# xuekt98/BBDM

Hardware: NVIDIA H100
Metric: denoising-steps/sec (UNet fwd) at 256^2 pixel-BBDM (higher is better)
Workload: dtype bf16x3 (split-bf16 tensor-core products, fp32 accumulate: fp32-class)

## Files before the change

bbdm_b200/csrc/winograd.cu:

```cuda
#include "common.cuh"
#include <cuda_fp16.h>
#include <stdlib.h>

namespace bbdm {

constexpr float WINO_WSCALE_FIXED = 256.0f;

__host__ __device__ inline float wino_wscale(uint32_t mbits) {
  if (mbits == 0) return WINO_WSCALE_FIXED;
  const int e = (int)(mbits >> 23) - 127;
  int k = 14 - (e + ((mbits & 0x7fffffu) != 0 ? 1 : 0));
  k = k < -100 ? -100 : (k > 100 ? 100 : k);
  float s = 1.0f;
  for (; k > 0; --k) s *= 2.0f;
  for (; k < 0; ++k) s *= 0.5f;
  return s;
}

template <int S>
__device__ __forceinline__ void wino_bt6(float* d) {
  const float d0 = d[0], d1 = d[S], d2 = d[2 * S], d3 = d[3 * S], d4 = d[4 * S], d5 = d[5 * S];
  d[0] = fmaf(4.0f, d0, fmaf(-5.0f, d2, d4));
  d[S] = fmaf(-4.0f, d1 + d2, d3 + d4);
  d[2 * S] = fmaf(4.0f, d1 - d2, d4 - d3);
  d[3 * S] = fmaf(2.0f, d3 - d1, d4 - d2);
  d[4 * S] = fmaf(2.0f, d1 - d3, d4 - d2);
  d[5 * S] = fmaf(4.0f, d1, fmaf(-5.0f, d3, d5));
}
template <int S, int T>
__host__ __device__ __forceinline__ void wino_at6(const float* m, float* y) {
  const float s12 = m[S] + m[2 * S], d12 = m[S] - m[2 * S];
  const float s34 = m[3 * S] + m[4 * S], d34 = m[3 * S] - m[4 * S];
  y[0] = (m[0] + s12) + s34;
  y[T] = fmaf(2.0f, d34, d12);
  y[2 * T] = fmaf(4.0f, s34, s12);
  y[3 * T] = fmaf(8.0f, d34, d12) + m[5 * S];
}

template <int S>
__device__ __forceinline__ void wino_bt8(float* d) {
  const float d0 = d[0], d1 = d[S], d2 = d[2 * S], d3 = d[3 * S], d4 = d[4 * S], d5 = d[5 * S], d6 = d[6 * S],
              d7 = d[7 * S];
  const float e1 = fmaf(-4.25f, d4, d2 + d6), o1 = fmaf(-4.25f, d3, d1 + d5);
  const float e3 = fmaf(0.25f, d2, fmaf(-1.25f, d4, d6)), o3 = fmaf(0.5f, d1, fmaf(-2.5f, d3, 2.0f * d5));
  const float e5 = fmaf(4.0f, d2, fmaf(-5.0f, d4, d6)), o5 = fmaf(2.0f, d1, fmaf(-2.5f, d3, 0.5f * d5));
  d[0] = fmaf(5.25f, d4 - d2, d0 - d6);
  d[S] = e1 + o1;
  d[2 * S] = e1 - o1;
  d[3 * S] = e3 + o3;
  d[4 * S] = e3 - o3;
  d[5 * S] = e5 + o5;
  d[6 * S] = e5 - o5;
  d[7 * S] = fmaf(5.25f, d3 - d5, d7 - d1);
}
template <int S, int T>
__host__ __device__ __forceinline__ void wino_at8(const float* m, float* y) {
  const float a = m[S] + m[2 * S], b = m[S] - m[2 * S];
  const float c = m[3 * S] + m[4 * S], d = m[3 * S] - m[4 * S];
  const float e = m[5 * S] + m[6 * S], f = m[5 * S] - m[6 * S];
  y[0] = ((m[0] + a) + c) + e;
  y[T] = fmaf(2.0f, d, fmaf(0.5f, f, b));
  y[2 * T] = fmaf(4.0f, c, fmaf(0.25f, e, a));
  y[3 * T] = fmaf(8.0f, d, fmaf(0.125f, f, b));
  y[4 * T] = fmaf(16.0f, c, fmaf(0.0625f, e, a));
  y[5 * T] = fmaf(32.0f, d, fmaf(0.03125f, f, b)) + m[7 * S];
}

__device__ __forceinline__ void split2_f16(float a, float b, uint32_t& hi, uint32_t& lo) {
  const __half2 h = __floats2half2_rn(a, b);
  const float2 hf = __half22float2(h);
  const __half2 l = __floats2half2_rn(a - hf.x, b - hf.y);
  hi = *reinterpret_cast<const uint32_t*>(&h);
  lo = *reinterpret_cast<const uint32_t*>(&l);
}

struct WinoInParams {
  const float* src1; int c1;
  const float* src2; int c2;
  int B, H, W, C, groups, cpg, th, tw;
  int64_t Mtot;
  const float* mean; const float* rstd; const float* gamma; const float* beta;
  const float* fscale; const float* fshift; int64_t fstride;
  int silu;
  __half* v_hi; __half* v_lo;
  __nv_bfloat16* raw_hi; __nv_bfloat16* raw_lo;
  __nv_bfloat16* act_hi; __nv_bfloat16* act_lo;
  unsigned long long* fault;
};

constexpr unsigned long long WINO6_RANGE_FAULT = 0xC0000000ull;

template <int VEC>
__global__ void __launch_bounds__(256)
wino_input_kernel(const WinoInParams p) {
  const int b = blockIdx.x / p.th, ty = blockIdx.x % p.th;
  const int c = (blockIdx.y * 256 + threadIdx.x) * VEC;
  if (c >= p.C) return;
  float sc[VEC], sh[VEC];
#pragma unroll
  for (int v = 0; v < VEC; ++v) {
    const int g = (c + v) / p.cpg;
    const float s0 = p.rstd[b * p.groups + g] * p.gamma[c + v];
    const float h0 = p.beta[c + v] - p.mean[b * p.groups + g] * s0;
    float f1 = 1.0f, f0 = 0.0f;
    if (p.fscale) { f1 = 1.0f + p.fscale[(int64_t)b * p.fstride + c + v]; f0 = p.fshift[(int64_t)b * p.fstride + c + v]; }
    sc[v] = s0 * f1;
    sh[v] = fmaf(h0, f1, f0);
  }
  const float* base;
  int cs, cc;
  if (c < p.c1) { base = p.src1; cs = p.c1; cc = c; } else { base = p.src2; cs = p.c2; cc = c - p.c1; }
  const int y0 = 4 * ty - 1;
  float act[VEC][36];
  auto fill = [&](int x0, int j0) {
#pragma unroll
    for (int i = 0; i < 6; ++i) {
      const int iy = y0 + i;
#pragma unroll
      for (int j = 0; j < 6; ++j) {
        if (j < j0) continue;
        const int ix = x0 + j;
        const bool in = iy >= 0 && iy < p.H && ix >= 0 && ix < p.W;
        float x[VEC];
#pragma unroll
        for (int v = 0; v < VEC; ++v) x[v] = 0.f;
        if (in) {
          const float* ptr = base + (((int64_t)b * p.H + iy) * p.W + ix) * cs + cc;
          if (VEC == 2) { const float2 t = *reinterpret_cast<const float2*>(ptr); x[0] = t.x; x[VEC - 1] = t.y; }
          else x[0] = *ptr;
        }
        if (p.raw_hi && i >= 1 && i <= 4 && j >= 2) {
          const int64_t off = (((int64_t)b * p.H + iy) * p.W + ix) * p.C + c;
          if (in) {
            if (VEC == 2) {
              uint32_t h, l;
              split2x(x[0], x[VEC - 1], h, l);
              *reinterpret_cast<uint32_t*>(p.raw_hi + off) = h;
              *reinterpret_cast<uint32_t*>(p.raw_lo + off) = l;
            } else {
              split_bf16(x[0], p.raw_hi[off], p.raw_lo[off]);
            }
          }
        } else if (p.raw_hi && i >= 1 && i <= 4 && j == 1 && j0 == 0 && in) {
          const int64_t off = (((int64_t)b * p.H + iy) * p.W + ix) * p.C + c;
          if (VEC == 2) {
            uint32_t h, l;
            split2x(x[0], x[VEC - 1], h, l);
            *reinterpret_cast<uint32_t*>(p.raw_hi + off) = h;
            *reinterpret_cast<uint32_t*>(p.raw_lo + off) = l;
          } else {
            split_bf16(x[0], p.raw_hi[off], p.raw_lo[off]);
          }
        }
#pragma unroll
        for (int v = 0; v < VEC; ++v) {
          float a = fmaf(x[v], sc[v], sh[v]);
          if (p.silu) a = __fdividef(a, 1.0f + __expf(-a));
          act[v][i * 6 + j] = in ? a : 0.f;
        }
      }
    }
  };
  for (int tx = 0; tx < p.tw; ++tx) {
    if (tx == 0) fill(-1, 0);
    else {
#pragma unroll
      for (int v = 0; v < VEC; ++v)
#pragma unroll
        for (int i = 0; i < 6; ++i) { act[v][i * 6] = act[v][i * 6 + 4]; act[v][i * 6 + 1] = act[v][i * 6 + 5]; }
      fill(4 * tx - 1, 2);
    }
    float t[VEC][36];
#pragma unroll
    for (int v = 0; v < VEC; ++v) {
#pragma unroll
      for (int q = 0; q < 36; ++q) t[v][q] = act[v][q];
#pragma unroll
      for (int j = 0; j < 6; ++j) wino_bt6<6>(t[v] + j);
#pragma unroll
      for (int i = 0; i < 6; ++i) wino_bt6<1>(t[v] + 6 * i);
    }
    const int64_t m = ((int64_t)b * p.th + ty) * p.tw + tx;
#pragma unroll
    for (int q = 0; q < 36; ++q) {
      const int64_t off = ((int64_t)q * p.Mtot + m) * p.C + c;
      if (VEC == 2) {
        uint32_t h, l;
        split2_f16(t[0][q], t[VEC - 1][q], h, l);
        *reinterpret_cast<uint32_t*>(p.v_hi + off) = h;
        *reinterpret_cast<uint32_t*>(p.v_lo + off) = l;
      } else {
        const __half h = __float2half_rn(t[0][q]);
        p.v_hi[off] = h;
        p.v_lo[off] = __float2half_rn(t[0][q] - __half2float(h));
      }
    }
  }
}

template <int T>
struct WinoIn {
  static constexpr int N = T + 2;
  static constexpr int CC = 64;
  static constexpr int TX = T == 4 ? 8 : 4;
  static constexpr int COLS = T * TX + 2;
  static constexpr int PATCH = N * COLS * CC;
  static constexpr size_t SMEM = 2 * (size_t)PATCH * sizeof(float);
};
static_assert(WinoIn<4>::SMEM == 2 * 6 * 34 * 64 * 4 && WinoIn<6>::SMEM * 2 <= 227 * 1024, "staged patch budget");

__device__ __forceinline__ void cp_async16(uint32_t saddr, const void* g) {
  asm volatile("cp.async.cg.shared.global [%0], [%1], 16;" ::"r"(saddr), "l"(g) : "memory");
}

template <int T>
__global__ void __launch_bounds__(256, 2)
wino_input_smem_kernel(const WinoInParams p) {
  using K = WinoIn<T>;
  constexpr int N = K::N, CC = K::CC, TX = K::TX, COLS = K::COLS;
  extern __shared__ __align__(16) float patch[];
  const int b = blockIdx.x / p.th, ty = blockIdx.x % p.th;
  const int cbase = blockIdx.y * CC;
  const float* base;
  int cs, cc0;
  if (cbase < p.c1) { base = p.src1; cs = p.c1; cc0 = cbase; } else { base = p.src2; cs = p.c2; cc0 = cbase - p.c1; }
  const int y0 = T * ty - 1;
  const int tid = threadIdx.x;
  const int ch4 = tid & 15;
  const int pix0 = tid >> 4;
  constexpr int NPIX = N * COLS;

  if constexpr (T == 6) {
    if (blockIdx.x == 0) {
      const int64_t tiles = (int64_t)p.B * p.th * p.tw;
      const int npad = (int)(p.Mtot - tiles);
      for (int k = tid; k < N * N * npad * CC; k += 256) {
        const int c = k % CC, r = (k / CC) % npad, q = k / (CC * npad);
        const int64_t off = ((int64_t)q * p.Mtot + tiles + r) * p.C + cbase + c;
        p.v_hi[off] = __float2half_rn(0.f);
        p.v_lo[off] = __float2half_rn(0.f);
      }
    }
  }

  float sc[4], sh[4];
#pragma unroll
  for (int v = 0; v < 4; ++v) {
    sc[v] = 1.0f; sh[v] = 0.0f;
    if (p.mean) {
      const int c = cbase + ch4 * 4 + v;
      const int g = c / p.cpg;
      const float s0 = p.rstd[b * p.groups + g] * p.gamma[c];
      const float h0 = p.beta[c] - p.mean[b * p.groups + g] * s0;
      float f1 = 1.0f, f0 = 0.0f;
      if (p.fscale) { f1 = 1.0f + p.fscale[(int64_t)b * p.fstride + c]; f0 = p.fshift[(int64_t)b * p.fstride + c]; }
      sc[v] = s0 * f1;
      sh[v] = fmaf(h0, f1, f0);
    }
  }
  const int nseg = (p.tw + TX - 1) / TX;
  const uint32_t patch_s = (uint32_t)__cvta_generic_to_shared(patch);

  auto stage = [&](int seg, int buf) {
    const int x0 = T * TX * seg - 1;
    int i = 0, j = pix0;
    for (int px = pix0; px < NPIX; px += 16, j += 16) {
      if (j >= COLS) { j -= COLS; ++i; }
      const int iy = y0 + i, ix = x0 + j;
      if (iy >= 0 && iy < p.H && ix >= 0 && ix < p.W)
        cp_async16(patch_s + (uint32_t)(((buf * NPIX + px) * CC + ch4 * 4) * 4),
                   base + (((int64_t)b * p.H + iy) * p.W + ix) * cs + cc0 + ch4 * 4);
    }
    asm volatile("cp.async.commit_group;" ::: "memory");
  };

  stage(0, 0);
  for (int seg = 0; seg < nseg; ++seg) {
    const int buf = seg & 1;
    if (seg + 1 < nseg) {
      stage(seg + 1, buf ^ 1);
      asm volatile("cp.async.wait_group 1;" ::: "memory");
    } else {
      asm volatile("cp.async.wait_group 0;" ::: "memory");
    }
    __syncthreads();
    float* pb = patch + buf * K::PATCH;
    const int x0 = T * TX * seg - 1;
    int i = 0, j = pix0;
    for (int px = pix0; px < NPIX; px += 16, j += 16) {
      if (j >= COLS) { j -= COLS; ++i; }
      const int iy = y0 + i, ix = x0 + j;
      float4* q = reinterpret_cast<float4*>(pb + px * CC + ch4 * 4);
      float4 a = make_float4(0.f, 0.f, 0.f, 0.f);
      if (iy >= 0 && iy < p.H && ix >= 0 && ix < p.W) {
        const float4 x = *q;
        if (p.raw_hi && i >= 1 && i <= T && j >= 1 && j <= T * TX) {
          uint2 h, l;
          split4(x, h, l);
          const int64_t off = (((int64_t)b * p.H + iy) * p.W + ix) * p.C + cbase + ch4 * 4;
          *reinterpret_cast<uint2*>(p.raw_hi + off) = h;
          *reinterpret_cast<uint2*>(p.raw_lo + off) = l;
        }
        a.x = fmaf(x.x, sc[0], sh[0]); a.y = fmaf(x.y, sc[1], sh[1]);
        a.z = fmaf(x.z, sc[2], sh[2]); a.w = fmaf(x.w, sc[3], sh[3]);
        if (p.silu) {
          a.x = __fdividef(a.x, 1.0f + __expf(-a.x)); a.y = __fdividef(a.y, 1.0f + __expf(-a.y));
          a.z = __fdividef(a.z, 1.0f + __expf(-a.z)); a.w = __fdividef(a.w, 1.0f + __expf(-a.w));
        }
        if (p.act_hi && i >= 1 && i <= T && j >= 1 && j <= T * TX) {
          uint2 h, l;
          split4(a, h, l);
          const int64_t off = (((int64_t)b * p.H + iy) * p.W + ix) * p.C + cbase + ch4 * 4;
          *reinterpret_cast<uint2*>(p.act_hi + off) = h;
          *reinterpret_cast<uint2*>(p.act_lo + off) = l;
        }
      }
      *q = a;
    }
    __syncthreads();
    const int64_t plane = p.Mtot * p.C;
    if constexpr (T == 4) {
      const int txl = tid >> 5, c0 = (tid & 31) * 2;
      const int tx = TX * seg + txl;
      if (tx < p.tw) {
        float t0[36], t1[36];
#pragma unroll
        for (int i = 0; i < 6; ++i)
#pragma unroll
          for (int j = 0; j < 6; ++j) {
            const float2 v = *reinterpret_cast<const float2*>(pb + ((i * COLS + 4 * txl + j) * CC + c0));
            t0[i * 6 + j] = v.x;
            t1[i * 6 + j] = v.y;
          }
#pragma unroll
        for (int j = 0; j < 6; ++j) { wino_bt6<6>(t0 + j); wino_bt6<6>(t1 + j); }
#pragma unroll
        for (int i = 0; i < 6; ++i) { wino_bt6<1>(t0 + 6 * i); wino_bt6<1>(t1 + 6 * i); }
        const int64_t m = ((int64_t)b * p.th + ty) * p.tw + tx;
        __half* ph = p.v_hi + m * p.C + cbase + c0;
        __half* pl = p.v_lo + m * p.C + cbase + c0;
#pragma unroll
        for (int q = 0; q < 36; ++q) {
          uint32_t h, l;
          split2_f16(t0[q], t1[q], h, l);
          *reinterpret_cast<uint32_t*>(ph) = h;
          *reinterpret_cast<uint32_t*>(pl) = l;
          ph += plane;
          pl += plane;
        }
      }
    } else {
      const int txl = tid >> 6, c = tid & 63;
      const int tx = TX * seg + txl;
      if (tx < p.tw) {
        float t[64];
#pragma unroll
        for (int i = 0; i < 8; ++i)
#pragma unroll
          for (int j = 0; j < 8; ++j) t[i * 8 + j] = pb[(i * COLS + 6 * txl + j) * CC + c];
#pragma unroll
        for (int j = 0; j < 8; ++j) wino_bt8<8>(t + j);
#pragma unroll
        for (int i = 0; i < 8; ++i) wino_bt8<1>(t + 8 * i);
        const int64_t m = ((int64_t)b * p.th + ty) * p.tw + tx;
        __half* ph = p.v_hi + m * p.C + cbase + c;
        __half* pl = p.v_lo + m * p.C + cbase + c;
        bool finite = true;
#pragma unroll
        for (int q = 0; q < 64; ++q) {
          const __half h = __float2half_rn(t[q]);
          finite &= fabsf(t[q]) < 65520.0f;
          *ph = h;
          *pl = __float2half_rn(t[q] - __half2float(h));
          ph += plane;
          pl += plane;
        }
        if (!finite) atomicExch(p.fault, WINO6_RANGE_FAULT | (unsigned)(p.C & 0xFFFFFFF));
      }
    }
    __syncthreads();
  }
}

struct WinoOutParams {
  const float* m; int64_t Mtot;
  const float* inv_wscale;
  int B, H, W, Cout, th, tw;
  const float* bias;
  const float* residual; int res_mode;
  float* out;
  float* stats;
};

template <int RES>
__host__ __device__ __forceinline__ void wino_output_tile(const WinoOutParams& p, int b, int ty, int tx, int c, float2 bv,
                                                          float inv, float& sum0, float& sum1, float& sq0, float& sq1) {
  const int64_t m = ((int64_t)b * p.th + ty) * p.tw + tx;
  float mx[36], my[36];
#pragma unroll
  for (int q = 0; q < 36; ++q) {
    const float2 v = *reinterpret_cast<const float2*>(p.m + ((int64_t)q * p.Mtot + m) * p.Cout + c);
    mx[q] = v.x; my[q] = v.y;
  }
  constexpr int NRES = RES == BBDM_RES_NONE ? 1 : (RES == BBDM_RES_UP2 ? 4 : 16);
  float2 rs[NRES];
  if constexpr (RES == BBDM_RES_SAME) {
#pragma unroll
    for (int i = 0; i < 4; ++i)
#pragma unroll
      for (int j = 0; j < 4; ++j)
        rs[i * 4 + j] = *reinterpret_cast<const float2*>(
            p.residual + (((int64_t)b * p.H + 4 * ty + i) * p.W + 4 * tx + j) * p.Cout + c);
  } else if constexpr (RES == BBDM_RES_UP2) {
#pragma unroll
    for (int i = 0; i < 2; ++i)
#pragma unroll
      for (int j = 0; j < 2; ++j)
        rs[i * 2 + j] = *reinterpret_cast<const float2*>(
            p.residual + (((int64_t)b * (p.H >> 1) + 2 * ty + i) * (p.W >> 1) + 2 * tx + j) * p.Cout + c);
  } else if constexpr (RES == BBDM_RES_DOWN2) {
    const int64_t W2 = (int64_t)p.W * 2;
#pragma unroll
    for (int i = 0; i < 4; ++i)
#pragma unroll
      for (int j = 0; j < 4; ++j) {
        const float* rp = p.residual + (((int64_t)b * p.H * 2 + (4 * ty + i) * 2) * W2 + (4 * tx + j) * 2) * p.Cout + c;
        const float2 t0 = *reinterpret_cast<const float2*>(rp), t1 = *reinterpret_cast<const float2*>(rp + p.Cout);
        const float2 t2 = *reinterpret_cast<const float2*>(rp + W2 * p.Cout);
        const float2 t3 = *reinterpret_cast<const float2*>(rp + (W2 + 1) * p.Cout);
        rs[i * 4 + j] = make_float2(0.25f * (((t0.x + t1.x) + t2.x) + t3.x), 0.25f * (((t0.y + t1.y) + t2.y) + t3.y));
      }
  }
  float tx4[24], ty4[24], yx[16], yy[16];
#pragma unroll
  for (int j = 0; j < 6; ++j) { wino_at6<6, 6>(mx + j, tx4 + j); wino_at6<6, 6>(my + j, ty4 + j); }
#pragma unroll
  for (int i = 0; i < 4; ++i) { wino_at6<1, 1>(tx4 + 6 * i, yx + 4 * i); wino_at6<1, 1>(ty4 + 6 * i, yy + 4 * i); }
#pragma unroll
  for (int i = 0; i < 4; ++i) {
    const int hh = 4 * ty + i;
#pragma unroll
    for (int j = 0; j < 4; ++j) {
      const int ww = 4 * tx + j;
      float r0 = fmaf(yx[i * 4 + j], inv, bv.x), r1 = fmaf(yy[i * 4 + j], inv, bv.y);
      if constexpr (RES == BBDM_RES_SAME || RES == BBDM_RES_DOWN2) {
        r0 += rs[i * 4 + j].x; r1 += rs[i * 4 + j].y;
      } else if constexpr (RES == BBDM_RES_UP2) {
        r0 += rs[(i >> 1) * 2 + (j >> 1)].x; r1 += rs[(i >> 1) * 2 + (j >> 1)].y;
      }
      *reinterpret_cast<float2*>(p.out + (((int64_t)b * p.H + hh) * p.W + ww) * p.Cout + c) = make_float2(r0, r1);
      sum0 += r0; sum1 += r1;
      sq0 = fmaf(r0, r0, sq0); sq1 = fmaf(r1, r1, sq1);
    }
  }
}

template <int RES>
__global__ void __launch_bounds__(256, 2)
wino_output_kernel(const WinoOutParams p) {
  __shared__ float red[8][64][2];
  const int cg = blockIdx.x, ty = blockIdx.y, b = blockIdx.z;
  const int lane = threadIdx.x & 31, tl = threadIdx.x >> 5;
  const int c = cg * 64 + lane * 2;
  float2 bv = make_float2(0.f, 0.f);
  if (p.bias) bv = *reinterpret_cast<const float2*>(p.bias + c);
  const float inv = p.inv_wscale ? __ldg(p.inv_wscale) : 1.0f / WINO_WSCALE_FIXED;
  float sum0 = 0.f, sum1 = 0.f, sq0 = 0.f, sq1 = 0.f;
  for (int tx = tl; tx < p.tw; tx += 8) wino_output_tile<RES>(p, b, ty, tx, c, bv, inv, sum0, sum1, sq0, sq1);
  if (p.stats) {
    red[tl][lane * 2][0] = sum0; red[tl][lane * 2][1] = sq0;
    red[tl][lane * 2 + 1][0] = sum1; red[tl][lane * 2 + 1][1] = sq1;
    __syncthreads();
    if (threadIdx.x < 64) {
      float a = 0.f, q = 0.f;
#pragma unroll
      for (int k = 0; k < 8; ++k) { a += red[k][threadIdx.x][0]; q += red[k][threadIdx.x][1]; }
      const int64_t prow = (int64_t)b * p.th + ty;
      *reinterpret_cast<float2*>(p.stats + (prow * p.Cout + cg * 64 + threadIdx.x) * 2) = make_float2(a, q);
    }
  }
}

template <int RES>
__host__ __device__ __forceinline__ void wino6_output_tile(const WinoOutParams& p, int b, int ty, int tx, int c, float bv,
                                                           float inv, float& sum, float& sq) {
  const int64_t m = ((int64_t)b * p.th + ty) * p.tw + tx;
  float mm[64];
#pragma unroll
  for (int q = 0; q < 64; ++q) mm[q] = p.m[((int64_t)q * p.Mtot + m) * p.Cout + c];
  float t6[48], y[36];
#pragma unroll
  for (int j = 0; j < 8; ++j) wino_at8<8, 8>(mm + j, t6 + j);
#pragma unroll
  for (int i = 0; i < 6; ++i) wino_at8<1, 1>(t6 + 8 * i, y + 6 * i);
  const int h0 = 6 * ty, w0 = 6 * tx;
  float rup[RES == BBDM_RES_UP2 ? 9 : 1];
  if constexpr (RES == BBDM_RES_UP2) {
    const int H2 = p.H >> 1, W2 = p.W >> 1;
#pragma unroll
    for (int i = 0; i < 3; ++i)
#pragma unroll
      for (int j = 0; j < 3; ++j)
        rup[i * 3 + j] = 3 * ty + i < H2 && 3 * tx + j < W2
                             ? p.residual[(((int64_t)b * H2 + 3 * ty + i) * W2 + 3 * tx + j) * p.Cout + c] : 0.f;
  }
  const int64_t pix0 = ((int64_t)b * p.H + h0) * p.W + w0;
#pragma unroll
  for (int i0 = 0; i0 < 6; i0 += 3) {
    float rs[18];
#pragma unroll
    for (int i = 0; i < 3; ++i)
#pragma unroll
      for (int j = 0; j < 6; ++j) {
        rs[i * 6 + j] = 0.f;
        if (h0 + i0 + i >= p.H || w0 + j >= p.W) continue;
        if constexpr (RES == BBDM_RES_SAME) {
          rs[i * 6 + j] = p.residual[(pix0 + (int64_t)(i0 + i) * p.W + j) * p.Cout + c];
        } else if constexpr (RES == BBDM_RES_DOWN2) {
          const int64_t W2 = (int64_t)p.W * 2;
          const float* rp = p.residual + (((int64_t)b * p.H * 2 + (h0 + i0 + i) * 2) * W2 + (w0 + j) * 2) * p.Cout + c;
          rs[i * 6 + j] = 0.25f * (((rp[0] + rp[p.Cout]) + rp[W2 * p.Cout]) + rp[(W2 + 1) * p.Cout]);
        }
      }
#pragma unroll
    for (int i = 0; i < 3; ++i)
#pragma unroll
      for (int j = 0; j < 6; ++j) {
        if (h0 + i0 + i >= p.H || w0 + j >= p.W) continue;
        float r = fmaf(y[(i0 + i) * 6 + j], inv, bv);
        if constexpr (RES == BBDM_RES_SAME || RES == BBDM_RES_DOWN2) r += rs[i * 6 + j];
        else if constexpr (RES == BBDM_RES_UP2) r += rup[((i0 + i) >> 1) * 3 + (j >> 1)];
        p.out[(pix0 + (int64_t)(i0 + i) * p.W + j) * p.Cout + c] = r;
        sum += r;
        sq = fmaf(r, r, sq);
      }
  }
}

template <int RES>
__global__ void __launch_bounds__(256, RES == BBDM_RES_SAME || RES == BBDM_RES_DOWN2 ? 1 : 2)
wino6_output_kernel(const WinoOutParams p) {
  __shared__ float red[4][64][2];
  const int cg = blockIdx.x, ty = blockIdx.y, b = blockIdx.z;
  const int cl = threadIdx.x & 63, tl = threadIdx.x >> 6;
  const int c = cg * 64 + cl;
  const float bv = p.bias ? p.bias[c] : 0.f;
  const float inv = p.inv_wscale ? __ldg(p.inv_wscale) : 1.0f / WINO_WSCALE_FIXED;
  float sum = 0.f, sq = 0.f;
  for (int tx = tl; tx < p.tw; tx += 4) wino6_output_tile<RES>(p, b, ty, tx, c, bv, inv, sum, sq);
  if (p.stats) {
    red[tl][cl][0] = sum; red[tl][cl][1] = sq;
    __syncthreads();
    if (threadIdx.x < 64) {
      float a = 0.f, q = 0.f;
#pragma unroll
      for (int k = 0; k < 4; ++k) { a += red[k][threadIdx.x][0]; q += red[k][threadIdx.x][1]; }
      const int64_t prow = (int64_t)b * p.th + ty;
      *reinterpret_cast<float2*>(p.stats + (prow * p.Cout + cg * 64 + threadIdx.x) * 2) = make_float2(a, q);
    }
  }
}

__global__ void __launch_bounds__(256)
wino_wmax_kernel(const float* __restrict__ w, int64_t n, uint32_t* __restrict__ wmax) {
  uint32_t m = 0;
  for (int64_t i = (int64_t)blockIdx.x * blockDim.x + threadIdx.x; i < n; i += (int64_t)gridDim.x * blockDim.x)
    m = max(m, __float_as_uint(fabsf(w[i])));
#pragma unroll
  for (int o = 16; o > 0; o >>= 1) m = max(m, __shfl_xor_sync(0xffffffffu, m, o));
  if ((threadIdx.x & 31) == 0 && m) atomicMax(wmax, m);
}

__global__ void wino_wscale_store_kernel(float* inv) {
  *inv = 1.0f / wino_wscale(__float_as_uint(*inv));
}

template <int T>
__device__ __forceinline__ void wino_g(double g0, double g1, double g2, double* u) {
  if constexpr (T == 4) {
    u[0] = g0 / 4.0;
    u[1] = -(g0 + g1 + g2) / 6.0;
    u[2] = -(g0 - g1 + g2) / 6.0;
    u[3] = g0 / 24.0 + g1 / 12.0 + g2 / 6.0;
    u[4] = g0 / 24.0 - g1 / 12.0 + g2 / 6.0;
    u[5] = g2;
  } else {
    u[0] = g0;
    u[1] = -2.0 * (g0 + g1 + g2) / 9.0;
    u[2] = -2.0 * (g0 - g1 + g2) / 9.0;
    u[3] = g0 / 90.0 + g1 / 45.0 + 2.0 * g2 / 45.0;
    u[4] = g0 / 90.0 - g1 / 45.0 + 2.0 * g2 / 45.0;
    u[5] = 32.0 * g0 / 45.0 + 16.0 * g1 / 45.0 + 8.0 * g2 / 45.0;
    u[6] = 32.0 * g0 / 45.0 - 16.0 * g1 / 45.0 + 8.0 * g2 / 45.0;
    u[7] = g2;
  }
}

template <int T>
__global__ void __launch_bounds__(256)
wino_weight_kernel(const float* __restrict__ w, int Cout, int Cin, int dgrad, const uint32_t* __restrict__ wmax,
                   __half* __restrict__ u_hi, __half* __restrict__ u_lo) {
  constexpr int N = T + 2;
  const int64_t n = (int64_t)Cout * Cin;
  const double s = wmax ? (double)wino_wscale(*wmax) : (double)WINO_WSCALE_FIXED;
  for (int64_t idx = (int64_t)blockIdx.x * blockDim.x + threadIdx.x; idx < n; idx += (int64_t)gridDim.x * blockDim.x) {
    double g[3][3], t[N][3];
    int64_t src = idx;
    if (dgrad) { const int64_t ci = idx / Cout, co = idx - ci * Cout; src = co * Cin + ci; }
#pragma unroll
    for (int i = 0; i < 9; ++i) {
      const int k = dgrad ? 8 - i : i;
      g[i / 3][i % 3] = (double)w[src * 9 + k];
    }
#pragma unroll
    for (int j = 0; j < 3; ++j) {
      double u[N];
      wino_g<T>(g[0][j], g[1][j], g[2][j], u);
#pragma unroll
      for (int i = 0; i < N; ++i) t[i][j] = u[i];
    }
#pragma unroll
    for (int i = 0; i < N; ++i) {
      double u[N];
      wino_g<T>(t[i][0], t[i][1], t[i][2], u);
#pragma unroll
      for (int j = 0; j < N; ++j) {
        const float v = (float)(u[j] * s);
        const __half h = __float2half_rn(v);
        const __half l = __float2half_rn(v - __half2float(h));
        const int64_t off = (int64_t)(i * N + j) * n + idx;
        u_hi[off] = h;
        u_lo[off] = l;
      }
    }
  }
}

}

using namespace bbdm;

namespace {

template <int T>
int wino_geometry_t(int B, int H, int W, int* tiles_h, int* tiles_w, int64_t* tiles_total, int* eligible) {
  BBDM_REQUIRE(B > 0 && H > 0 && W > 0, "wino_geometry: bad shape");
  const int th = T == 4 ? H / 4 : (H + 5) / 6, tw = T == 4 ? W / 4 : (W + 5) / 6;
  int64_t mtot = (int64_t)B * th * tw;
  if (T == 6) mtot = mtot < 128 ? 128 : (mtot + 15) / 16 * 16;
  if (tiles_h) *tiles_h = th;
  if (tiles_w) *tiles_w = tw;
  if (tiles_total) *tiles_total = mtot;
  const bool aligned = T == 6 || (H % 4 == 0 && W % 4 == 0);
  if (eligible) *eligible = (aligned && mtot % 16 == 0 && mtot >= 128) ? 1 : 0;
  return BBDM_OK;
}

template <int T>
int wino_input_t(const BbdmWinoInputArgs* a, void* stream) {
  BBDM_REQUIRE(a && a->src1 && a->v_hi && a->v_lo, "wino_input: null args");
  WinoInParams p;
  p.src1 = a->src1; p.c1 = a->c1;
  p.src2 = a->src2; p.c2 = a->src2 ? a->c2 : 0;
  p.B = a->B; p.H = a->H; p.W = a->W;
  p.C = p.c1 + p.c2;
  p.groups = a->groups;
  if (T == 4)
    BBDM_REQUIRE(p.B > 0 && p.H > 0 && p.W > 0 && p.H % 4 == 0 && p.W % 4 == 0, "wino_input: H, W must be multiples of 4");
  else
    BBDM_REQUIRE(p.B > 0 && p.H > 0 && p.W > 0, "wino6_input: bad shape");
  BBDM_REQUIRE(p.c1 % 2 == 0 && p.c2 % 2 == 0 && p.C > 0, "wino_input: channel counts must be even");
  if (a->mean) {
    BBDM_REQUIRE(a->rstd && a->gamma && a->beta && p.groups > 0 && p.C % p.groups == 0, "wino_input: incomplete GroupNorm args");
  } else {
    BBDM_REQUIRE(!a->silu && !a->film_scale, "wino_input: identity mode (mean == NULL) takes no activation / FiLM");
    if (p.groups <= 0) p.groups = 1;
  }
  BBDM_REQUIRE((a->act_hi == nullptr) == (a->act_lo == nullptr), "wino_input: act hi/lo must come in pairs");
  BBDM_REQUIRE((a->film_scale == nullptr) == (a->film_shift == nullptr), "wino_input: film scale/shift mismatch");
  BBDM_REQUIRE((a->raw_hi == nullptr) == (a->raw_lo == nullptr), "wino_input: raw hi/lo must come in pairs");
  p.cpg = p.C / p.groups;
  wino_geometry_t<T>(p.B, p.H, p.W, &p.th, &p.tw, &p.Mtot, nullptr);
  p.mean = a->mean; p.rstd = a->rstd; p.gamma = a->gamma; p.beta = a->beta;
  p.fscale = a->film_scale; p.fshift = a->film_shift; p.fstride = a->film_stride;
  p.silu = a->silu;
  p.v_hi = (__half*)a->v_hi; p.v_lo = (__half*)a->v_lo;
  p.raw_hi = (__nv_bfloat16*)a->raw_hi; p.raw_lo = (__nv_bfloat16*)a->raw_lo;
  p.act_hi = (__nv_bfloat16*)a->act_hi; p.act_lo = (__nv_bfloat16*)a->act_lo;
  p.fault = nullptr;
  if (T == 6) {
    p.fault = device_fault_ptr();
    BBDM_REQUIRE(p.fault != nullptr, "wino6_input: device fault word unavailable");
  }
  const bool smem_only = a->mean == nullptr || a->act_hi != nullptr;
  const int64_t ctas = (int64_t)p.B * p.th;
  BBDM_REQUIRE(ctas < (1ll << 31), "wino_input: too many tile rows");
  constexpr int CC = WinoIn<T>::CC;
  static int vec = -1;
  if (vec < 0) { const char* e = getenv("BBDM_WINO_IN_VEC"); vec = e ? (atoi(e) == 2 ? 2 : 1) : 0; }
  if ((T == 6 || vec == 0) && p.c1 % CC == 0 && p.c2 % CC == 0) {
    static DeviceOnce configured;
    if (configured.need()) {
      BBDM_CUDA_CHECK(cudaFuncSetAttribute(wino_input_smem_kernel<T>, cudaFuncAttributeMaxDynamicSharedMemorySize,
                                           (int)WinoIn<T>::SMEM));
      configured.mark();
    }
    dim3 grid((unsigned)ctas, p.C / CC);
    wino_input_smem_kernel<T><<<grid, 256, WinoIn<T>::SMEM, (cudaStream_t)stream>>>(p);
  } else if (T == 6) {
    BBDM_REQUIRE(false, "wino6_input: channel counts must be multiples of 64");
  } else if (smem_only) {
    BBDM_REQUIRE(false, "wino_input: identity mode / act planes need channel counts that are multiples of 64");
  } else if (vec == 2 || (vec == 0 && p.c1 % 2 == 0 && p.c2 % 2 == 0)) {
    dim3 grid((unsigned)ctas, (p.C / 2 + 255) / 256);
    wino_input_kernel<2><<<grid, 256, 0, (cudaStream_t)stream>>>(p);
  } else {
    dim3 grid((unsigned)ctas, (p.C + 255) / 256);
    wino_input_kernel<1><<<grid, 256, 0, (cudaStream_t)stream>>>(p);
  }
  BBDM_LAUNCH_CHECK();
  return BBDM_OK;
}

template <int T>
int wino_output_t(const BbdmWinoOutputArgs* a, void* stream) {
  BBDM_REQUIRE(a && a->m && a->out, "wino_output: null args");
  WinoOutParams p;
  p.m = a->m; p.inv_wscale = a->inv_wscale;
  p.B = a->B; p.H = a->H; p.W = a->W; p.Cout = a->Cout;
  if (T == 4)
    BBDM_REQUIRE(p.B > 0 && p.B <= 65535 && p.H > 0 && p.W > 0 && p.H % 4 == 0 && p.W % 4 == 0,
                 "wino_output: H, W must be multiples of 4 (B <= 65535)");
  else
    BBDM_REQUIRE(p.B > 0 && p.B <= 65535 && p.H > 0 && p.W > 0, "wino6_output: bad shape (B <= 65535)");
  BBDM_REQUIRE(p.Cout > 0 && p.Cout % 64 == 0, "wino_output: Cout %% 64 != 0");
  BBDM_REQUIRE(a->res_mode >= 0 && a->res_mode <= 3 && (a->res_mode == 0 || a->residual), "wino_output: bad residual");
  if (a->res_mode == BBDM_RES_UP2) BBDM_REQUIRE(p.H % 2 == 0 && p.W % 2 == 0, "wino_output: RES_UP2 needs even H, W");
  wino_geometry_t<T>(p.B, p.H, p.W, &p.th, &p.tw, &p.Mtot, nullptr);
  BBDM_REQUIRE(p.th <= 65535, "wino_output: too many tile rows");
  p.bias = a->bias; p.residual = a->residual; p.res_mode = a->res_mode;
  p.out = a->out; p.stats = a->stats_partial;
  dim3 grid(p.Cout / 64, p.th, p.B);
  cudaStream_t st = (cudaStream_t)stream;
  if constexpr (T == 4) {
    switch (p.res_mode) {
      case BBDM_RES_SAME: wino_output_kernel<BBDM_RES_SAME><<<grid, 256, 0, st>>>(p); break;
      case BBDM_RES_UP2: wino_output_kernel<BBDM_RES_UP2><<<grid, 256, 0, st>>>(p); break;
      case BBDM_RES_DOWN2: wino_output_kernel<BBDM_RES_DOWN2><<<grid, 256, 0, st>>>(p); break;
      default: wino_output_kernel<BBDM_RES_NONE><<<grid, 256, 0, st>>>(p); break;
    }
  } else {
    switch (p.res_mode) {
      case BBDM_RES_SAME: wino6_output_kernel<BBDM_RES_SAME><<<grid, 256, 0, st>>>(p); break;
      case BBDM_RES_UP2: wino6_output_kernel<BBDM_RES_UP2><<<grid, 256, 0, st>>>(p); break;
      case BBDM_RES_DOWN2: wino6_output_kernel<BBDM_RES_DOWN2><<<grid, 256, 0, st>>>(p); break;
      default: wino6_output_kernel<BBDM_RES_NONE><<<grid, 256, 0, st>>>(p); break;
    }
  }
  BBDM_LAUNCH_CHECK();
  return BBDM_OK;
}

template <int T>
int wino_pack_weight_t(const float* w, int Cout, int Cin, int dgrad, void* u_hi, void* u_lo, float* inv_wscale,
                       void* stream) {
  BBDM_REQUIRE(w && u_hi && u_lo && Cout > 0 && Cin > 0, "wino_pack_weight: bad args");
  cudaStream_t st = (cudaStream_t)stream;
  const int64_t n = (int64_t)Cout * Cin;
  uint32_t* wmax = reinterpret_cast<uint32_t*>(inv_wscale);
  if (wmax) {
    BBDM_CUDA_CHECK(cudaMemsetAsync(wmax, 0, sizeof(uint32_t), st));
    int64_t g = (n * 9 + 255) / 256;
    if (g > (int64_t)num_sms() * 8) g = (int64_t)num_sms() * 8;
    wino_wmax_kernel<<<(unsigned)g, 256, 0, st>>>(w, n * 9, wmax);
  }
  int64_t g = (n + 255) / 256;
  if (g > (int64_t)num_sms() * 16) g = (int64_t)num_sms() * 16;
  wino_weight_kernel<T><<<(unsigned)g, 256, 0, st>>>(w, Cout, Cin, dgrad, wmax, (__half*)u_hi, (__half*)u_lo);
  if (wmax) wino_wscale_store_kernel<<<1, 1, 0, st>>>(inv_wscale);
  BBDM_LAUNCH_CHECK();
  return BBDM_OK;
}

}

extern "C" {

int bbdm_wino_geometry(int B, int H, int W, int* tiles_h, int* tiles_w, int64_t* tiles_total, int* eligible) {
  return wino_geometry_t<4>(B, H, W, tiles_h, tiles_w, tiles_total, eligible);
}
int bbdm_wino_input(const BbdmWinoInputArgs* a, void* stream) { return wino_input_t<4>(a, stream); }
int bbdm_wino_output(const BbdmWinoOutputArgs* a, void* stream) { return wino_output_t<4>(a, stream); }
int bbdm_wino_pack_weight(const float* w, int Cout, int Cin, int dgrad, void* u_hi, void* u_lo, float* inv_wscale,
                          void* stream) {
  return wino_pack_weight_t<4>(w, Cout, Cin, dgrad, u_hi, u_lo, inv_wscale, stream);
}

int bbdm_wino6_geometry(int B, int H, int W, int* tiles_h, int* tiles_w, int64_t* tiles_total, int* eligible) {
  return wino_geometry_t<6>(B, H, W, tiles_h, tiles_w, tiles_total, eligible);
}
int bbdm_wino6_input(const BbdmWinoInputArgs* a, void* stream) { return wino_input_t<6>(a, stream); }
int bbdm_wino6_output(const BbdmWinoOutputArgs* a, void* stream) { return wino_output_t<6>(a, stream); }
int bbdm_wino6_pack_weight(const float* w, int Cout, int Cin, int dgrad, void* u_hi, void* u_lo, float* inv_wscale,
                           void* stream) {
  return wino_pack_weight_t<6>(w, Cout, Cin, dgrad, u_hi, u_lo, inv_wscale, stream);
}

}
```

Before: 5.558.

## Prefetch F(6,3) Winograd output residuals via cp.async and flatten input grid

The F(6,3) output kernel now issues the residual loads for SAME and DOWN2 modes as asynchronous cp.async copies into per-thread shared-memory slots before the output transform. This lets those loads overlap the inverse-transform arithmetic and frees the registers that held them, so launch bounds rise to two CTAs per SM. Separately, the F(6,3) input kernel uses a 1D grid with the channel chunk as the fastest-varying index, which changes CTA ordering and spreads pad zeroing across the first chunk of CTAs. The cost is up to 72 KB of dynamic shared memory per CTA in DOWN2 mode, which may limit residency, and clamped (duplicated) residual loads at image edges.

Result: no change. 5.610, median of 6 (+0.9%).

```diff
diff --git a/bbdm_b200/csrc/winograd.cu b/bbdm_b200/csrc/winograd.cu
--- a/bbdm_b200/csrc/winograd.cu
+++ b/bbdm_b200/csrc/winograd.cu
@@ -219,8 +219,10 @@
   using K = WinoIn<T>;
   constexpr int N = K::N, CC = K::CC, TX = K::TX, COLS = K::COLS;
   extern __shared__ __align__(16) float patch[];
-  const int b = blockIdx.x / p.th, ty = blockIdx.x % p.th;
-  const int cbase = blockIdx.y * CC;
+  const int nchunk = p.C / CC;
+  const int b = T == 6 ? (int)(blockIdx.x / nchunk) / p.th : blockIdx.x / p.th;
+  const int ty = T == 6 ? (int)(blockIdx.x / nchunk) % p.th : blockIdx.x % p.th;
+  const int cbase = (T == 6 ? (int)(blockIdx.x % nchunk) : blockIdx.y) * CC;
   const float* base;
   int cs, cc0;
   if (cbase < p.c1) { base = p.src1; cs = p.c1; cc0 = cbase; } else { base = p.src2; cs = p.c2; cc0 = cbase - p.c1; }
@@ -231,7 +233,7 @@
   constexpr int NPIX = N * COLS;
 
   if constexpr (T == 6) {
-    if (blockIdx.x == 0) {
+    if (blockIdx.x < nchunk) {
       const int64_t tiles = (int64_t)p.B * p.th * p.tw;
       const int npad = (int)(p.Mtot - tiles);
       for (int k = tid; k < N * N * npad * CC; k += 256) {
@@ -481,9 +483,53 @@
   }
 }
 
+__host__ __device__ __forceinline__ void wino6_res_fetch(float* slot, const float* g) {
+#ifdef __CUDA_ARCH__
+  asm volatile("cp.async.ca.shared.global [%0], [%1], 4;" ::"r"((uint32_t)__cvta_generic_to_shared(slot)), "l"(g)
+               : "memory");
+#else
+  *slot = *g;
+#endif
+}
+__host__ __device__ __forceinline__ void wino6_res_wait() {
+#ifdef __CUDA_ARCH__
+  asm volatile("cp.async.wait_all;" ::: "memory");
+#endif
+}
+template <int RES>
+constexpr int wino6_res_slots() { return RES == BBDM_RES_SAME ? 36 : (RES == BBDM_RES_DOWN2 ? 72 : 0); }
+
 template <int RES>
 __host__ __device__ __forceinline__ void wino6_output_tile(const WinoOutParams& p, int b, int ty, int tx, int c, float bv,
-                                                           float inv, float& sum, float& sq) {
+                                                           float inv, float& sum, float& sq, float* st = nullptr,
+                                                           int sst = 1) {
+#ifndef __CUDA_ARCH__
+  float host_slots[wino6_res_slots<RES>() > 0 ? wino6_res_slots<RES>() : 1];
+  if (st == nullptr) { st = host_slots; sst = 1; }
+#endif
+  const int h0 = 6 * ty, w0 = 6 * tx;
+  const int64_t pix0 = ((int64_t)b * p.H + h0) * p.W + w0;
+  auto fetch = [&](int i0, int n) {
+    for (int i = 0; i < n; ++i)
+#pragma unroll
+      for (int j = 0; j < 6; ++j) {
+        if constexpr (RES == BBDM_RES_SAME) {
+          const int hh = min(h0 + i0 + i, p.H - 1), ww = min(w0 + j, p.W - 1);
+          wino6_res_fetch(st + ((i0 + i) * 6 + j) * sst, p.residual + (((int64_t)b * p.H + hh) * p.W + ww) * p.Cout + c);
+        } else if constexpr (RES == BBDM_RES_DOWN2) {
+          if (h0 + i0 + i >= p.H || w0 + j >= p.W) continue;
+          const int64_t W2 = (int64_t)p.W * 2;
+          const float* rp = p.residual + (((int64_t)b * p.H * 2 + (h0 + i0 + i) * 2) * W2 + (w0 + j) * 2) * p.Cout + c;
+          float* s = st + (i * 6 + j) * 4 * sst;
+          wino6_res_fetch(s, rp);
+          wino6_res_fetch(s + sst, rp + p.Cout);
+          wino6_res_fetch(s + 2 * sst, rp + W2 * p.Cout);
+          wino6_res_fetch(s + 3 * sst, rp + (W2 + 1) * p.Cout);
+        }
+      }
+  };
+  if constexpr (RES == BBDM_RES_SAME) fetch(0, 6);
+  else if constexpr (RES == BBDM_RES_DOWN2) fetch(0, 3);
   const int64_t m = ((int64_t)b * p.th + ty) * p.tw + tx;
   float mm[64];
 #pragma unroll
@@ -493,7 +539,6 @@
   for (int j = 0; j < 8; ++j) wino_at8<8, 8>(mm + j, t6 + j);
 #pragma unroll
   for (int i = 0; i < 6; ++i) wino_at8<1, 1>(t6 + 8 * i, y + 6 * i);
-  const int h0 = 6 * ty, w0 = 6 * tx;
   float rup[RES == BBDM_RES_UP2 ? 9 : 1];
   if constexpr (RES == BBDM_RES_UP2) {
     const int H2 = p.H >> 1, W2 = p.W >> 1;
@@ -504,32 +549,26 @@
         rup[i * 3 + j] = 3 * ty + i < H2 && 3 * tx + j < W2
                              ? p.residual[(((int64_t)b * H2 + 3 * ty + i) * W2 + 3 * tx + j) * p.Cout + c] : 0.f;
   }
-  const int64_t pix0 = ((int64_t)b * p.H + h0) * p.W + w0;
 #pragma unroll
   for (int i0 = 0; i0 < 6; i0 += 3) {
-    float rs[18];
-#pragma unroll
-    for (int i = 0; i < 3; ++i)
-#pragma unroll
-      for (int j = 0; j < 6; ++j) {
-        rs[i * 6 + j] = 0.f;
-        if (h0 + i0 + i >= p.H || w0 + j >= p.W) continue;
-        if constexpr (RES == BBDM_RES_SAME) {
-          rs[i * 6 + j] = p.residual[(pix0 + (int64_t)(i0 + i) * p.W + j) * p.Cout + c];
-        } else if constexpr (RES == BBDM_RES_DOWN2) {
-          const int64_t W2 = (int64_t)p.W * 2;
-          const float* rp = p.residual + (((int64_t)b * p.H * 2 + (h0 + i0 + i) * 2) * W2 + (w0 + j) * 2) * p.Cout + c;
-          rs[i * 6 + j] = 0.25f * (((rp[0] + rp[p.Cout]) + rp[W2 * p.Cout]) + rp[(W2 + 1) * p.Cout]);
-        }
-      }
+    if constexpr (RES == BBDM_RES_DOWN2) {
+      if (i0 == 3) fetch(3, 3);
+    }
+    if constexpr (RES == BBDM_RES_SAME || RES == BBDM_RES_DOWN2) wino6_res_wait();
 #pragma unroll
     for (int i = 0; i < 3; ++i)
 #pragma unroll
       for (int j = 0; j < 6; ++j) {
         if (h0 + i0 + i >= p.H || w0 + j >= p.W) continue;
         float r = fmaf(y[(i0 + i) * 6 + j], inv, bv);
-        if constexpr (RES == BBDM_RES_SAME || RES == BBDM_RES_DOWN2) r += rs[i * 6 + j];
-        else if constexpr (RES == BBDM_RES_UP2) r += rup[((i0 + i) >> 1) * 3 + (j >> 1)];
+        if constexpr (RES == BBDM_RES_SAME) {
+          r += st[((i0 + i) * 6 + j) * sst];
+        } else if constexpr (RES == BBDM_RES_DOWN2) {
+          const float* s = st + (i * 6 + j) * 4 * sst;
+          r += 0.25f * (((s[0] + s[sst]) + s[2 * sst]) + s[3 * sst]);
+        } else if constexpr (RES == BBDM_RES_UP2) {
+          r += rup[((i0 + i) >> 1) * 3 + (j >> 1)];
+        }
         p.out[(pix0 + (int64_t)(i0 + i) * p.W + j) * p.Cout + c] = r;
         sum += r;
         sq = fmaf(r, r, sq);
@@ -538,16 +577,18 @@
 }
 
 template <int RES>
-__global__ void __launch_bounds__(256, RES == BBDM_RES_SAME || RES == BBDM_RES_DOWN2 ? 1 : 2)
+__global__ void __launch_bounds__(256, 2)
 wino6_output_kernel(const WinoOutParams p) {
   __shared__ float red[4][64][2];
+  extern __shared__ float res_slots[];
   const int cg = blockIdx.x, ty = blockIdx.y, b = blockIdx.z;
   const int cl = threadIdx.x & 63, tl = threadIdx.x >> 6;
   const int c = cg * 64 + cl;
   const float bv = p.bias ? p.bias[c] : 0.f;
   const float inv = p.inv_wscale ? __ldg(p.inv_wscale) : 1.0f / WINO_WSCALE_FIXED;
   float sum = 0.f, sq = 0.f;
-  for (int tx = tl; tx < p.tw; tx += 4) wino6_output_tile<RES>(p, b, ty, tx, c, bv, inv, sum, sq);
+  for (int tx = tl; tx < p.tw; tx += 4)
+    wino6_output_tile<RES>(p, b, ty, tx, c, bv, inv, sum, sq, res_slots + threadIdx.x, 256);
   if (p.stats) {
     red[tl][cl][0] = sum; red[tl][cl][1] = sq;
     __syncthreads();
@@ -705,7 +746,8 @@
                                            (int)WinoIn<T>::SMEM));
       configured.mark();
     }
-    dim3 grid((unsigned)ctas, p.C / CC);
+    if (T == 6) BBDM_REQUIRE(ctas * (p.C / CC) < (1ll << 31), "wino6_input: too many CTAs");
+    const dim3 grid = T == 6 ? dim3((unsigned)(ctas * (p.C / CC))) : dim3((unsigned)ctas, p.C / CC);
     wino_input_smem_kernel<T><<<grid, 256, WinoIn<T>::SMEM, (cudaStream_t)stream>>>(p);
   } else if (T == 6) {
     BBDM_REQUIRE(false, "wino6_input: channel counts must be multiples of 64");
@@ -750,10 +792,20 @@
       default: wino_output_kernel<BBDM_RES_NONE><<<grid, 256, 0, st>>>(p); break;
     }
   } else {
+    constexpr size_t same_smem = wino6_res_slots<BBDM_RES_SAME>() * 256 * sizeof(float);
+    constexpr size_t down2_smem = wino6_res_slots<BBDM_RES_DOWN2>() * 256 * sizeof(float);
+    static DeviceOnce configured;
+    if (configured.need()) {
+      BBDM_CUDA_CHECK(cudaFuncSetAttribute(wino6_output_kernel<BBDM_RES_SAME>,
+                                           cudaFuncAttributeMaxDynamicSharedMemorySize, (int)same_smem));
+      BBDM_CUDA_CHECK(cudaFuncSetAttribute(wino6_output_kernel<BBDM_RES_DOWN2>,
+                                           cudaFuncAttributeMaxDynamicSharedMemorySize, (int)down2_smem));
+      configured.mark();
+    }
     switch (p.res_mode) {
-      case BBDM_RES_SAME: wino6_output_kernel<BBDM_RES_SAME><<<grid, 256, 0, st>>>(p); break;
+      case BBDM_RES_SAME: wino6_output_kernel<BBDM_RES_SAME><<<grid, 256, same_smem, st>>>(p); break;
       case BBDM_RES_UP2: wino6_output_kernel<BBDM_RES_UP2><<<grid, 256, 0, st>>>(p); break;
-      case BBDM_RES_DOWN2: wino6_output_kernel<BBDM_RES_DOWN2><<<grid, 256, 0, st>>>(p); break;
+      case BBDM_RES_DOWN2: wino6_output_kernel<BBDM_RES_DOWN2><<<grid, 256, down2_smem, st>>>(p); break;
       default: wino6_output_kernel<BBDM_RES_NONE><<<grid, 256, 0, st>>>(p); break;
     }
   }
```
